# changzy00/pytorch-attention

Measured on AMD Instinct MI355X. Metric: forward images/sec through one step (+ ms/block), B=256 per GPU, 224x224-derived shapes, higher is better.
Workload: dtype f32/f16; 1 GPU; north-star step: C2 SE+CBAM+ECA, C3 ViT-Attn, C4 CSWin s1-4 + XCABlock + XCA, DA x2, Mixer, C5 ViT-Base fwd; B=256/GPU; precision=fp16-mfma, ranks_seen=1, gather=none (single rank), batch_per_gpu=256, parallelism=batch-shard x1, dist_backend=none, rccl_self_test=not run (single rank), distinct_gpus=1, full=off: --full adds calibration, roofline, per-block and CPU-baseline figures

## Files before the change

pytorch-attention_amd/csrc/attn.hip:

```cpp
#include "common.h"
#include "mma.h"
#include "bufops.h"
#include <type_traits>

namespace {

struct AttnArgs {
    const void* qkv;
    void* out;
    const float* lepe_w;
    const float* lepe_b;
    int L, Ctot, c0, heads;
    int koff, voff, oc0;
    int reso, Hsp, Wsp, nWx, nwin;
    int T;
    unsigned wsp_magic;
    float scale;
    int pre_scale;
};

struct AttnPair {
    AttnArgs a0, a1;
    int split;
};
struct AttnPairRg : AttnPair {
    unsigned* ovf;
};
struct AttnPairQ : AttnPair {
    int q_tiles, q_rows;
    int out_rows;
};
template <bool IO16, bool QLIM = false>
using attn_kargs = typename std::conditional<QLIM, AttnPairQ, typename std::conditional<IO16, AttnPair, AttnPairRg>::type>::type;
template <bool IO16>
const attn_kargs<IO16>& attn_pick(const AttnPairRg& p) { return p; }

#ifndef MI355_ATTN_FMA_SM
#define MI355_ATTN_FMA_SM 1
#endif
template <int PREC, int D, int KT, bool LEPE, bool IO16, int NW, int OCC = 1, int TFULL = -1, bool QLIM = false>
__global__ __launch_bounds__(NW * 64, OCC) void win_attn_kernel(const attn_kargs<IO16, QLIM> pr) {
    static_assert(!QLIM || (IO16 && !LEPE), "the query limit exists for the plain 16-bit-I/O core");
    constexpr bool FMA_SM = MI355_ATTN_FMA_SM != 0;
    const int lid = xcd_contiguous_block();
    const bool second = lid >= pr.split;
    const AttnArgs a = second ? pr.a1 : pr.a0;
    constexpr int NTHR = NW * 64;
    static_assert(!IO16 || PREC != 0, "16-bit I/O exists for the fp16 / bf16 operand modes only");
    using M_ = Mma<PREC>;
    using v8 = typename M_::v8;
    using v4 = typename M_::v4;
    using el = typename M_::e;
    constexpr int NS = M_::NSPLIT;
    constexpr int TK = KT * 16;
    constexpr int KP = D + 8;
    constexpr int VP = TK + 4;
    constexpr bool RG = !IO16 && PREC == 1;
    float rgm = 0.f;
    constexpr int OP = IO16 ? D + 8 : D + 4;
    constexpr int K_EL = TK * KP, V_EL = D * VP;
    using slab_t = typename std::conditional<IO16, unsigned short, float>::type;
    __shared__ __attribute__((aligned(16))) unsigned short s_k[NS * K_EL];
    __shared__ __attribute__((aligned(16))) unsigned short s_v[NS * V_EL];
    __shared__ __attribute__((aligned(16))) slab_t s_o[NW * 16 * OP];

    const int t = threadIdx.x, lane = t & 63, wave = t >> 6;
    int bid = lid - (second ? pr.split : 0);
    const int head = bid % a.heads; bid /= a.heads;
    const int win = bid % a.nwin;
    const int b = bid / a.nwin;
    const int T = a.T;
    const int wy0 = (win / a.nWx) * a.Hsp, wx0 = (win % a.nWx) * a.Wsp;
    const int ch0 = a.c0 + head * D;
    const int och0 = a.oc0 + head * D;
    const long row3 = 3L * a.Ctot;
    using gel = typename std::conditional<IO16, el, float>::type;
    const gel* base = static_cast<const gel*>(a.qkv) + (long)b * a.L * row3 + ch0;
    auto srow = [&](int s) { return a.Wsp == 1 ? s : (int)__umulhi((unsigned)s, a.wsp_magic); };
    auto tok = [&](int s) { const int r = srow(s); return (wy0 + r) * a.reso + wx0 + (s - r * a.Wsp); };

    const int l15 = lane & 15, g = lane >> 4;
    int nqt = (T + 15) >> 4;
    int qmax = T;
    if constexpr (QLIM) {
        nqt = pr.q_tiles < nqt ? pr.q_tiles : nqt;
        qmax = pr.q_rows < T ? pr.q_rows : T;
    }
    int orows = a.L;
    if constexpr (QLIM) orows = pr.out_rows;
    constexpr int NQ = (KT + NW - 1) / NW;
    const rsrc_t img_rs = make_rsrc(IO16 ? static_cast<const void*>(base) : nullptr, IO16 ? (bufops_u32)((long)a.L * row3 * sizeof(gel)) : 0u);
    auto ld16 = [&](bool live, int token, int el_off) -> v8 {
        const bufops_u32 off = live ? (bufops_u32)((token * (int)row3 + el_off) * 2) : OOB;
        return __builtin_bit_cast(v8, __builtin_amdgcn_raw_buffer_load_b128(img_rs, off, 0, 0));
    };
    v8 qraw[IO16 ? NQ : 1][D / 32];
    if constexpr (IO16) {
#pragma unroll
        for (int iq = 0; iq < NQ; ++iq) {
            const int qs = (wave + iq * NW) * 16 + l15;
            const int tq = tok(qs < T ? qs : 0);
            const bool ql = QLIM ? (qs < qmax && wave + iq * NW < nqt) : qs < T;
#pragma unroll
            for (int ks = 0; ks < D / 32; ++ks) qraw[iq][ks] = ld16(ql, tq, ks * 32 + g * 8);
        }
    }
    __shared__ float s_lw[LEPE ? D * 10 : 1];
    if constexpr (LEPE) {
        for (int q = t; q < D * 10; q += NTHR) {
            const int c = q / 10, i = q - c * 10;
            s_lw[q] = i < 9 ? a.lepe_w[(long)(head * D + c) * 9 + i] : a.lepe_b[head * D + c];
        }
    }

    constexpr int D4 = D / 4;
    if constexpr (IO16) {
        constexpr int D8 = D / 8;
        constexpr int NKI = (TK * D8 + NTHR - 1) / NTHR, NVI = ((TK / 4) * D8 + NTHR - 1) / NTHR;
        v8 kreg[NKI];
        v8 vreg[NVI][4];
#pragma unroll
        for (int it = 0; it < NKI; ++it) {
            const int idx = t + it * NTHR, key = idx / D8, d8 = idx % D8;
            const bool live = idx < TK * D8 && key < T;
            kreg[it] = ld16(live, tok(live ? key : 0), a.koff + d8 * 8);
        }
#pragma unroll
        for (int it = 0; it < NVI; ++it) {
            const int idx = t + it * NTHR, kg = idx / D8, d8 = idx % D8;
#pragma unroll
            for (int j = 0; j < 4; ++j) {
                const int key = kg * 4 + j;
                const bool live = idx < (TK / 4) * D8 && key < T;
                vreg[it][j] = ld16(live, tok(live ? key : 0), a.voff + d8 * 8);
            }
        }
#pragma unroll
        for (int it = 0; it < NKI; ++it) {
            const int idx = t + it * NTHR, key = idx / D8, d8 = idx % D8;
            if (idx < TK * D8) *reinterpret_cast<v8*>(s_k + key * KP + d8 * 8) = kreg[it];
        }
#pragma unroll
        for (int it = 0; it < NVI; ++it) {
            const int idx = t + it * NTHR, kg = idx / D8, d8 = idx % D8;
            if (idx < (TK / 4) * D8) {
#pragma unroll
                for (int q = 0; q < 8; ++q)
                    *reinterpret_cast<v4*>(s_v + (d8 * 8 + q) * VP + kg * 4) =
                        v4{vreg[it][0][q], vreg[it][1][q], vreg[it][2][q], vreg[it][3][q]};
            }
        }
    } else {
    for (int idx = t; idx < TK * D4; idx += NTHR) {
        const int key = idx / D4, d4 = idx % D4;
        f4 v = {0.f, 0.f, 0.f, 0.f};
        if (key < T) v = *reinterpret_cast<const f4*>(base + (long)tok(key) * row3 + a.koff + d4 * 4);
        if constexpr (RG) rgm = rg_absmax4(rgm, v);
        const v4 h = M_::cvt(v);
        *reinterpret_cast<v4*>(s_k + key * KP + d4 * 4) = h;
        if constexpr (NS == 2) *reinterpret_cast<v4*>(s_k + K_EL + key * KP + d4 * 4) = M_::cvt_lo(v, h);
    }
    for (int idx = t; idx < (TK / 4) * D4; idx += NTHR) {
        const int kg = idx / D4, d4 = idx % D4;
        f4 r[4];
#pragma unroll
        for (int j = 0; j < 4; ++j) {
            const int key = kg * 4 + j;
            r[j] = f4{0.f, 0.f, 0.f, 0.f};
            if (key < T) r[j] = *reinterpret_cast<const f4*>(base + (long)tok(key) * row3 + a.voff + d4 * 4);
            if constexpr (RG) rgm = rg_absmax4(rgm, r[j]);
        }
        const f4 c[4] = {{r[0].x, r[1].x, r[2].x, r[3].x}, {r[0].y, r[1].y, r[2].y, r[3].y},
                         {r[0].z, r[1].z, r[2].z, r[3].z}, {r[0].w, r[1].w, r[2].w, r[3].w}};
#pragma unroll
        for (int q = 0; q < 4; ++q) {
            const v4 h = M_::cvt(c[q]);
            *reinterpret_cast<v4*>(s_v + (d4 * 4 + q) * VP + kg * 4) = h;
            if constexpr (NS == 2) *reinterpret_cast<v4*>(s_v + V_EL + (d4 * 4 + q) * VP + kg * 4) = M_::cvt_lo(c[q], h);
        }
    }
    }
    __shared__ unsigned short s_tap[LEPE ? TK * 9 : 1];
    if constexpr (LEPE) {
        for (int q = t; q < NS * D; q += NTHR) s_v[(q / D) * V_EL + (q % D) * VP + TK] = 0;
        for (int q = t; q < T * 9; q += NTHR) {
            const int slot = q / 9, tap = q - slot * 9;
            const int ty = srow(slot), tx = slot - ty * a.Wsp;
            const int yy = ty + tap / 3 - 1, xx = tx + tap % 3 - 1;
            s_tap[q] = (unsigned short)(((yy >= 0 && yy < a.Hsp && xx >= 0 && xx < a.Wsp) ? yy * a.Wsp + xx : TK) * 2);
        }
    }
    __syncthreads();

    slab_t* slab = s_o + wave * 16 * OP;
#pragma unroll
    for (int iq = 0; iq < NQ; ++iq) {
        const int qt = wave + iq * NW;
        if (qt >= nqt) break;
        const int qs = qt * 16 + l15;
        v8 qf[D / 32][NS];
        {
            const gel* qrow = base + (long)tok(qs < T ? qs : 0) * row3;
#pragma unroll
            for (int ks = 0; ks < D / 32; ++ks) {
                f4 lo4 = {0.f, 0.f, 0.f, 0.f}, hi4 = {0.f, 0.f, 0.f, 0.f};
                if constexpr (IO16) {
                    const v8 raw = qraw[iq][ks];
                    if (!a.pre_scale) { qf[ks][0] = raw; continue; }
                    lo4 = f4{(float)raw[0], (float)raw[1], (float)raw[2], (float)raw[3]};
                    hi4 = f4{(float)raw[4], (float)raw[5], (float)raw[6], (float)raw[7]};
                } else if (qs < T) {
                    lo4 = *reinterpret_cast<const f4*>(qrow + ks * 32 + g * 8);
                    hi4 = *reinterpret_cast<const f4*>(qrow + ks * 32 + g * 8 + 4);
                }
                if (a.pre_scale) { lo4 = lo4 * a.scale; hi4 = hi4 * a.scale; }
                if constexpr (RG) rgm = rg_absmax4(rg_absmax4(rgm, lo4), hi4);
                const v4 h0 = M_::cvt(lo4), h1 = M_::cvt(hi4);
                qf[ks][0] = v8{h0.x, h0.y, h0.z, h0.w, h1.x, h1.y, h1.z, h1.w};
                if constexpr (NS == 2) {
                    const v4 e0 = M_::cvt_lo(lo4, h0), e1 = M_::cvt_lo(hi4, h1);
                    qf[ks][1] = v8{e0.x, e0.y, e0.z, e0.w, e1.x, e1.y, e1.z, e1.w};
                }
            }
        }
        f4 o[D / 16];
        float sum;
        const f4 zero4 = {0.f, 0.f, 0.f, 0.f};
        f4 s[KT];
#pragma unroll
        for (int kt = 0; kt < KT; ++kt) {
            f4 acc = zero4;
            if (kt < TFULL || kt * 16 < T) {
#pragma unroll
                for (int ks = 0; ks < D / 32; ++ks) {
                    v8 kf[NS];
#pragma unroll
                    for (int sp = 0; sp < NS; ++sp)
                        kf[sp] = *reinterpret_cast<const v8*>(s_k + sp * K_EL + (kt * 16 + l15) * KP + ks * 32 + g * 8);
                    acc = mma_step<PREC>(kf, qf[ks], acc);
                }
            }
            s[kt] = acc;
        }
        const float post = (a.pre_scale ? 1.0f : a.scale) * 1.44269504088896340736f;
        float m = -INFINITY;
        sum = 0.f;
        if constexpr (PREC != 0 && FMA_SM) {
#pragma unroll
            for (int kt = 0; kt < KT; ++kt)
#pragma unroll
                for (int r = 0; r < 4; ++r) {
                    const int key = kt * 16 + g * 4 + r;
                    const float v = (kt < TFULL || key < T) ? s[kt][r] : -INFINITY;
                    s[kt][r] = v;
                    m = fmaxf(m, v);
                }
            m = fmaxf(m, __shfl_xor(m, 16, WAVE));
            m = fmaxf(m, __shfl_xor(m, 32, WAVE));
            const float mneg = -(m * post);
#pragma unroll
            for (int kt = 0; kt < KT; ++kt)
#pragma unroll
                for (int r = 0; r < 4; ++r) {
                    s[kt][r] = __builtin_amdgcn_exp2f(__builtin_fmaf(s[kt][r], post, mneg));
                }
        } else {
#pragma unroll
            for (int kt = 0; kt < KT; ++kt)
#pragma unroll
                for (int r = 0; r < 4; ++r) {
                    const int key = kt * 16 + g * 4 + r;
                    const float v = (kt < TFULL || key < T) ? s[kt][r] * post : -INFINITY;
                    s[kt][r] = v;
                    m = fmaxf(m, v);
                }
            m = fmaxf(m, __shfl_xor(m, 16, WAVE));
            m = fmaxf(m, __shfl_xor(m, 32, WAVE));
#pragma unroll
            for (int kt = 0; kt < KT; ++kt)
#pragma unroll
                for (int r = 0; r < 4; ++r) {
                    const float p = __builtin_amdgcn_exp2f(s[kt][r] - m);
                    s[kt][r] = p;
                    sum += p;
                }
        }
        if constexpr (!(PREC != 0 && FMA_SM)) {
            sum += __shfl_xor(sum, 16, WAVE);
            sum += __shfl_xor(sum, 32, WAVE);
        }
#pragma unroll
        for (int nt = 0; nt < D / 16; ++nt) o[nt] = zero4;
        f4 osum = zero4;
        typedef typename M_::e el1_t;
        const v8 ones = v8{(el1_t)1.0f, (el1_t)1.0f, (el1_t)1.0f, (el1_t)1.0f, (el1_t)1.0f, (el1_t)1.0f, (el1_t)1.0f, (el1_t)1.0f};
#pragma unroll
        for (int kb = 0; kb < KT / 2; ++kb) {
            if (2 * kb < TFULL || kb * 32 < T) {
                v8 pf[NS];
                {
                    const f4 p0 = s[2 * kb], p1 = s[2 * kb + 1];
                    const v4 h0 = M_::cvt(p0), h1 = M_::cvt(p1);
                    pf[0] = v8{h0.x, h0.y, h0.z, h0.w, h1.x, h1.y, h1.z, h1.w};
                    if constexpr (NS == 2) {
                        const v4 e0 = M_::cvt_lo(p0, h0), e1 = M_::cvt_lo(p1, h1);
                        pf[1] = v8{e0.x, e0.y, e0.z, e0.w, e1.x, e1.y, e1.z, e1.w};
                    }
                }
#pragma unroll
                for (int nt = 0; nt < D / 16; ++nt) {
                    v8 vf[NS];
#pragma unroll
                    for (int sp = 0; sp < NS; ++sp) {
                        const unsigned short* vr = s_v + sp * V_EL + (nt * 16 + l15) * VP + kb * 32 + g * 4;
                        const v4 a0 = *reinterpret_cast<const v4*>(vr);
                        const v4 a1 = *reinterpret_cast<const v4*>(vr + 16);
                        vf[sp] = v8{a0.x, a0.y, a0.z, a0.w, a1.x, a1.y, a1.z, a1.w};
                    }
                    o[nt] = mma_step<PREC>(vf, pf, o[nt]);
                }
                if constexpr (PREC != 0 && FMA_SM) osum = M_::mma(ones, pf[0], osum);
            }
        }
        if constexpr (PREC != 0 && FMA_SM) sum = osum.x;
        const float inv = __builtin_amdgcn_rcpf(sum);
        int off[LEPE ? 9 : 1];
        bool qlive = false;
        if constexpr (LEPE) {
            const int qslot = qt * 16 + l15;
            qlive = qslot < T;
            const unsigned short* tp = s_tap + (qlive ? qslot : 0) * 9;
#pragma unroll
            for (int i = 0; i < 9; ++i) off[i] = tp[i];
        }
#pragma unroll
        for (int nt = 0; nt < D / 16; ++nt) {
            f4 val = o[nt] * inv;
            if constexpr (LEPE) {
                if (qlive) {
#pragma unroll
                    for (int r = 0; r < 4; ++r) {
                        const int d = nt * 16 + g * 4 + r;
                        const float* lwp = s_lw + d * 10;
                        const char* vrow = reinterpret_cast<const char*>(s_v + d * VP);
                        float acc = lwp[9];
#pragma unroll
                        for (int i = 0; i < 9; ++i) {
                            float vv = (float)(*reinterpret_cast<const el*>(vrow + off[i]));
                            if constexpr (NS == 2) vv += (float)(*reinterpret_cast<const el*>(vrow + V_EL * 2 + off[i]));
                            acc = __builtin_fmaf(lwp[i], vv, acc);
                        }
                        val[r] += acc;
                    }
                }
            }
            if constexpr (IO16) *reinterpret_cast<v4*>(slab + l15 * OP + nt * 16 + g * 4) = M_::cvt(val);
            else *reinterpret_cast<f4*>(slab + l15 * OP + nt * 16 + g * 4) = val;
        }
        __builtin_amdgcn_wave_barrier();
        __builtin_amdgcn_fence(__ATOMIC_ACQ_REL, "wavefront");
        if constexpr (IO16) {
            constexpr int LPR = D / 8, RPI = 64 / LPR;
#pragma unroll
            for (int it = 0; it < 16 / RPI; ++it) {
                const int r = it * RPI + lane / LPR, c8 = (lane % LPR) * 8;
                const int qslot = qt * 16 + r;
                if (QLIM ? qslot < qmax : qslot < T)
                    *reinterpret_cast<v8*>(static_cast<gel*>(a.out) + ((long)b * orows + tok(qslot)) * a.Ctot + och0 + c8) =
                        *reinterpret_cast<const v8*>(slab + r * OP + c8);
            }
        } else {
            constexpr int LPR = D / 4, RPI = 64 / LPR;
#pragma unroll
            for (int it = 0; it < 16 / RPI; ++it) {
                const int r = it * RPI + lane / LPR, c4 = (lane % LPR) * 4;
                const int qslot = qt * 16 + r;
                if (qslot < T)
                    *reinterpret_cast<f4*>(static_cast<gel*>(a.out) + ((long)b * a.L + tok(qslot)) * a.Ctot + och0 + c4) =
                        *reinterpret_cast<const f4*>(slab + r * OP + c4);
            }
        }
        __builtin_amdgcn_wave_barrier();
        __builtin_amdgcn_fence(__ATOMIC_ACQ_REL, "wavefront");
    }
    if constexpr (RG) rg_report(rgm, pr.ovf, 7u);
}

constexpr int LONG_KB = 8;
constexpr int LONG_TMAX = 512;
template <int PREC, int KT, bool IO16, int NW>
__global__ __launch_bounds__(NW * 64, 1) void win_attn_long_kernel(const attn_kargs<IO16> pr) {
    constexpr int D = 32, KB = LONG_KB;
    static_assert(!IO16 || PREC != 0, "16-bit I/O exists for the fp16 / bf16 operand modes only");
    static_assert(KT % 2 == 0 && KB % 2 == 0 && KT * 16 <= LONG_TMAX, "P.V consumes key tiles in pairs");
    const int lid = xcd_contiguous_block();
    const bool second = lid >= pr.split;
    const AttnArgs a = second ? pr.a1 : pr.a0;
    constexpr int NTHR = NW * 64;
    using M_ = Mma<PREC>;
    using v8 = typename M_::v8;
    using v4 = typename M_::v4;
    using el = typename M_::e;
    constexpr int NS = M_::NSPLIT;
    constexpr int TK = KT * 16;
    constexpr int KP = D + 8;
    constexpr int VP = TK + 4;
    static_assert((TK + 1) * 2 <= VP * 2 && VP * 2 < 65536, "tap byte offsets stay inside a V^T row");
    constexpr bool RG = !IO16 && PREC == 1;
    float rgm = 0.f;
    constexpr int OP = IO16 ? D + 8 : D + 4;
    constexpr int K_EL = TK * KP, V_EL = D * VP;
    using slab_t = typename std::conditional<IO16, unsigned short, float>::type;
    __shared__ __attribute__((aligned(16))) unsigned short s_k[NS * K_EL];
    __shared__ __attribute__((aligned(16))) unsigned short s_v[NS * V_EL];
    __shared__ __attribute__((aligned(16))) slab_t s_o[NW * 16 * OP];
    __shared__ float s_lw[D * 10];
    static_assert(sizeof(unsigned short) * NS * (K_EL + V_EL) + sizeof(slab_t) * NW * 16 * OP + sizeof(float) * D * 10 <= 163840,
                  "K, V^T, the output slab and the LePE weights share one workgroup's LDS");

    const int t = threadIdx.x, lane = t & 63, wave = t >> 6;
    int bid = lid - (second ? pr.split : 0);
    const int head = bid % a.heads; bid /= a.heads;
    const int win = bid % a.nwin;
    const int b = bid / a.nwin;
    const int T = a.T;
    const int wy0 = (win / a.nWx) * a.Hsp, wx0 = (win % a.nWx) * a.Wsp;
    const int ch0 = a.c0 + head * D;
    const int och0 = a.oc0 + head * D;
    const long row3 = 3L * a.Ctot;
    using gel = typename std::conditional<IO16, el, float>::type;
    const gel* base = static_cast<const gel*>(a.qkv) + (long)b * a.L * row3 + ch0;
    auto srow = [&](int s) { return a.Wsp == 1 ? s : (int)__umulhi((unsigned)s, a.wsp_magic); };
    auto tok = [&](int s) { const int r = srow(s); return (wy0 + r) * a.reso + wx0 + (s - r * a.Wsp); };

    const int l15 = lane & 15, g = lane >> 4;
    const int nqt = (T + 15) >> 4;
    const rsrc_t img_rs = make_rsrc(IO16 ? static_cast<const void*>(base) : nullptr, IO16 ? (bufops_u32)((long)a.L * row3 * sizeof(gel)) : 0u);
    auto ld16 = [&](bool live, int token, int el_off) -> v8 {
        const bufops_u32 off = live ? (bufops_u32)((token * (int)row3 + el_off) * 2) : OOB;
        return __builtin_bit_cast(v8, __builtin_amdgcn_raw_buffer_load_b128(img_rs, off, 0, 0));
    };
    const f4 zero4 = {0.f, 0.f, 0.f, 0.f};
    struct QF32 { f4 lo, hi; };
    using qraw_t = typename std::conditional<IO16, v8, QF32>::type;
    auto ldq = [&](int qt_) -> qraw_t {
        const int qs = qt_ * 16 + l15;
        const bool live = qs < T;
        const int tq = tok(live ? qs : 0);
        if constexpr (IO16) {
            return ld16(live, tq, g * 8);
        } else {
            QF32 r{zero4, zero4};
            if (live) {
                const float* qrow = base + (long)tq * row3 + g * 8;
                r.lo = *reinterpret_cast<const f4*>(qrow);
                r.hi = *reinterpret_cast<const f4*>(qrow + 4);
            }
            return r;
        }
    };
    qraw_t qnext = ldq(wave);
    for (int q = t; q < D * 10; q += NTHR) {
        const int c = q / 10, i = q - c * 10;
        s_lw[q] = i < 9 ? a.lepe_w[(long)(head * D + c) * 9 + i] : a.lepe_b[head * D + c];
    }

    constexpr int D4 = D / 4;
    if constexpr (IO16) {
        constexpr int D8 = D / 8;
        constexpr int NKI = (TK * D8 + NTHR - 1) / NTHR, NVI = ((TK / 4) * D8 + NTHR - 1) / NTHR;
        v8 kreg[NKI];
        v8 vreg[NVI][4];
#pragma unroll
        for (int it = 0; it < NKI; ++it) {
            const int idx = t + it * NTHR, key = idx / D8, d8 = idx % D8;
            const bool live = idx < TK * D8 && key < T;
            kreg[it] = ld16(live, tok(live ? key : 0), a.koff + d8 * 8);
        }
#pragma unroll
        for (int it = 0; it < NVI; ++it) {
            const int idx = t + it * NTHR, kg = idx / D8, d8 = idx % D8;
#pragma unroll
            for (int j = 0; j < 4; ++j) {
                const int key = kg * 4 + j;
                const bool live = idx < (TK / 4) * D8 && key < T;
                vreg[it][j] = ld16(live, tok(live ? key : 0), a.voff + d8 * 8);
            }
        }
#pragma unroll
        for (int it = 0; it < NKI; ++it) {
            const int idx = t + it * NTHR, key = idx / D8, d8 = idx % D8;
            if (idx < TK * D8) *reinterpret_cast<v8*>(s_k + key * KP + d8 * 8) = kreg[it];
        }
#pragma unroll
        for (int it = 0; it < NVI; ++it) {
            const int idx = t + it * NTHR, kg = idx / D8, d8 = idx % D8;
            if (idx < (TK / 4) * D8) {
#pragma unroll
                for (int q = 0; q < 8; ++q)
                    *reinterpret_cast<v4*>(s_v + (d8 * 8 + q) * VP + kg * 4) =
                        v4{vreg[it][0][q], vreg[it][1][q], vreg[it][2][q], vreg[it][3][q]};
            }
        }
    } else {
        for (int idx = t; idx < TK * D4; idx += NTHR) {
            const int key = idx / D4, d4 = idx % D4;
            f4 v = zero4;
            if (key < T) v = *reinterpret_cast<const f4*>(base + (long)tok(key) * row3 + a.koff + d4 * 4);
            if constexpr (RG) rgm = rg_absmax4(rgm, v);
            const v4 h = M_::cvt(v);
            *reinterpret_cast<v4*>(s_k + key * KP + d4 * 4) = h;
            if constexpr (NS == 2) *reinterpret_cast<v4*>(s_k + K_EL + key * KP + d4 * 4) = M_::cvt_lo(v, h);
        }
        for (int idx = t; idx < (TK / 4) * D4; idx += NTHR) {
            const int kg = idx / D4, d4 = idx % D4;
            f4 r[4];
#pragma unroll
            for (int j = 0; j < 4; ++j) {
                const int key = kg * 4 + j;
                r[j] = zero4;
                if (key < T) r[j] = *reinterpret_cast<const f4*>(base + (long)tok(key) * row3 + a.voff + d4 * 4);
                if constexpr (RG) rgm = rg_absmax4(rgm, r[j]);
            }
            const f4 c[4] = {{r[0].x, r[1].x, r[2].x, r[3].x}, {r[0].y, r[1].y, r[2].y, r[3].y},
                             {r[0].z, r[1].z, r[2].z, r[3].z}, {r[0].w, r[1].w, r[2].w, r[3].w}};
#pragma unroll
            for (int q = 0; q < 4; ++q) {
                const v4 h = M_::cvt(c[q]);
                *reinterpret_cast<v4*>(s_v + (d4 * 4 + q) * VP + kg * 4) = h;
                if constexpr (NS == 2) *reinterpret_cast<v4*>(s_v + V_EL + (d4 * 4 + q) * VP + kg * 4) = M_::cvt_lo(c[q], h);
            }
        }
    }
    for (int q = t; q < NS * D; q += NTHR) s_v[(q / D) * V_EL + (q % D) * VP + TK] = 0;
    __syncthreads();

    slab_t* slab = s_o + wave * 16 * OP;
    const float post = (a.pre_scale ? 1.0f : a.scale) * 1.44269504088896340736f;
    for (int qt = wave; qt < nqt; qt += NW) {
        const qraw_t qr = qnext;
        qnext = ldq(qt + NW);
        v8 qf[NS];
        {
            f4 lo4, hi4;
            if constexpr (IO16) {
                lo4 = f4{(float)qr[0], (float)qr[1], (float)qr[2], (float)qr[3]};
                hi4 = f4{(float)qr[4], (float)qr[5], (float)qr[6], (float)qr[7]};
            } else {
                lo4 = qr.lo; hi4 = qr.hi;
            }
            if (a.pre_scale) { lo4 = lo4 * a.scale; hi4 = hi4 * a.scale; }
            if constexpr (RG) rgm = rg_absmax4(rg_absmax4(rgm, lo4), hi4);
            const v4 h0 = M_::cvt(lo4), h1 = M_::cvt(hi4);
            qf[0] = v8{h0.x, h0.y, h0.z, h0.w, h1.x, h1.y, h1.z, h1.w};
            if constexpr (NS == 2) {
                const v4 e0 = M_::cvt_lo(lo4, h0), e1 = M_::cvt_lo(hi4, h1);
                qf[1] = v8{e0.x, e0.y, e0.z, e0.w, e1.x, e1.y, e1.z, e1.w};
            }
        }
        f4 o[D / 16] = {zero4, zero4};
        float m = -INFINITY, sum = 0.f;
        typedef typename M_::e el1_t;
        const v8 ones = v8{(el1_t)1.0f, (el1_t)1.0f, (el1_t)1.0f, (el1_t)1.0f, (el1_t)1.0f, (el1_t)1.0f, (el1_t)1.0f, (el1_t)1.0f};
        for (int kb0 = 0; kb0 * 16 < T; kb0 += KB) {
            f4 s[KB];
#pragma unroll
            for (int kt = 0; kt < KB; ++kt) {
                f4 acc = zero4;
                if ((kb0 + kt) * 16 < T) {
                    v8 kf[NS];
#pragma unroll
                    for (int sp = 0; sp < NS; ++sp)
                        kf[sp] = *reinterpret_cast<const v8*>(s_k + sp * K_EL + ((kb0 + kt) * 16 + l15) * KP + g * 8);
                    acc = mma_step<PREC>(kf, qf, acc);
                }
                s[kt] = acc;
            }
            float mb = -INFINITY;
#pragma unroll
            for (int kt = 0; kt < KB; ++kt)
#pragma unroll
                for (int r = 0; r < 4; ++r) {
                    const int key = (kb0 + kt) * 16 + g * 4 + r;
                    const float sc = PREC != 0 ? s[kt][r] : s[kt][r] * post;
                    const float v = key < T ? sc : -INFINITY;
                    s[kt][r] = v;
                    mb = fmaxf(mb, v);
                }
            mb = fmaxf(mb, __shfl_xor(mb, 16, WAVE));
            mb = fmaxf(mb, __shfl_xor(mb, 32, WAVE));
            const float mn = fmaxf(m, mb);
            float alpha, bsum = 0.f;
            if constexpr (PREC != 0) {
                const float mneg = -(mn * post);
                alpha = m == -INFINITY ? 0.f : __builtin_amdgcn_exp2f(__builtin_fmaf(m, post, mneg));
#pragma unroll
                for (int kt = 0; kt < KB; ++kt)
#pragma unroll
                    for (int r = 0; r < 4; ++r) s[kt][r] = __builtin_amdgcn_exp2f(__builtin_fmaf(s[kt][r], post, mneg));
            } else {
                alpha = m == -INFINITY ? 0.f : __builtin_amdgcn_exp2f(m - mn);
#pragma unroll
                for (int kt = 0; kt < KB; ++kt)
#pragma unroll
                    for (int r = 0; r < 4; ++r) {
                        const float p = __builtin_amdgcn_exp2f(s[kt][r] - mn);
                        s[kt][r] = p;
                        bsum += p;
                    }
            }
            m = mn;
#pragma unroll
            for (int nt = 0; nt < D / 16; ++nt) o[nt] = o[nt] * alpha;
            f4 osum = zero4;
#pragma unroll
            for (int kb = 0; kb < KB / 2; ++kb) {
                if ((kb0 + 2 * kb) * 16 < T) {
                    v8 pf[NS];
                    {
                        const f4 p0 = s[2 * kb], p1 = s[2 * kb + 1];
                        const v4 h0 = M_::cvt(p0), h1 = M_::cvt(p1);
                        pf[0] = v8{h0.x, h0.y, h0.z, h0.w, h1.x, h1.y, h1.z, h1.w};
                        if constexpr (NS == 2) {
                            const v4 e0 = M_::cvt_lo(p0, h0), e1 = M_::cvt_lo(p1, h1);
                            pf[1] = v8{e0.x, e0.y, e0.z, e0.w, e1.x, e1.y, e1.z, e1.w};
                        }
                    }
#pragma unroll
                    for (int nt = 0; nt < D / 16; ++nt) {
                        v8 vf[NS];
#pragma unroll
                        for (int sp = 0; sp < NS; ++sp) {
                            const unsigned short* vr = s_v + sp * V_EL + (nt * 16 + l15) * VP + (kb0 + 2 * kb) * 16 + g * 4;
                            const v4 a0 = *reinterpret_cast<const v4*>(vr);
                            const v4 a1 = *reinterpret_cast<const v4*>(vr + 16);
                            vf[sp] = v8{a0.x, a0.y, a0.z, a0.w, a1.x, a1.y, a1.z, a1.w};
                        }
                        o[nt] = mma_step<PREC>(vf, pf, o[nt]);
                    }
                    if constexpr (PREC != 0) osum = M_::mma(ones, pf[0], osum);
                }
            }
            if constexpr (PREC != 0) bsum = osum.x;
            sum = sum * alpha + bsum;
        }
        if constexpr (PREC == 0) {
            sum += __shfl_xor(sum, 16, WAVE);
            sum += __shfl_xor(sum, 32, WAVE);
        }
        const float inv = __builtin_amdgcn_rcpf(sum);
        const int qslot = qt * 16 + l15;
        const bool qlive = qslot < T;
        int off[9];
        {
            const int ty = srow(qlive ? qslot : 0), tx = (qlive ? qslot : 0) - ty * a.Wsp;
#pragma unroll
            for (int i = 0; i < 9; ++i) {
                const int yy = ty + i / 3 - 1, xx = tx + i % 3 - 1;
                off[i] = ((yy >= 0 && yy < a.Hsp && xx >= 0 && xx < a.Wsp) ? yy * a.Wsp + xx : TK) * 2;
            }
        }
#pragma unroll
        for (int nt = 0; nt < D / 16; ++nt) {
            f4 val = o[nt] * inv;
            if (qlive) {
#pragma unroll
                for (int r = 0; r < 4; ++r) {
                    const int d = nt * 16 + g * 4 + r;
                    const float* lwp = s_lw + d * 10;
                    const char* vrow = reinterpret_cast<const char*>(s_v + d * VP);
                    float acc = lwp[9];
#pragma unroll
                    for (int i = 0; i < 9; ++i) {
                        float vv = (float)(*reinterpret_cast<const el*>(vrow + off[i]));
                        if constexpr (NS == 2) vv += (float)(*reinterpret_cast<const el*>(vrow + V_EL * 2 + off[i]));
                        acc = __builtin_fmaf(lwp[i], vv, acc);
                    }
                    val[r] += acc;
                }
            }
            if constexpr (IO16) *reinterpret_cast<v4*>(slab + l15 * OP + nt * 16 + g * 4) = M_::cvt(val);
            else *reinterpret_cast<f4*>(slab + l15 * OP + nt * 16 + g * 4) = val;
        }
        __builtin_amdgcn_wave_barrier();
        __builtin_amdgcn_fence(__ATOMIC_ACQ_REL, "wavefront");
        if constexpr (IO16) {
            constexpr int LPR = D / 8, RPI = 64 / LPR;
#pragma unroll
            for (int it = 0; it < 16 / RPI; ++it) {
                const int r = it * RPI + lane / LPR, c8 = (lane % LPR) * 8;
                const int qs = qt * 16 + r;
                if (qs < T)
                    *reinterpret_cast<v8*>(static_cast<gel*>(a.out) + ((long)b * a.L + tok(qs)) * a.Ctot + och0 + c8) =
                        *reinterpret_cast<const v8*>(slab + r * OP + c8);
            }
        } else {
            constexpr int LPR = D / 4, RPI = 64 / LPR;
#pragma unroll
            for (int it = 0; it < 16 / RPI; ++it) {
                const int r = it * RPI + lane / LPR, c4 = (lane % LPR) * 4;
                const int qs = qt * 16 + r;
                if (qs < T)
                    *reinterpret_cast<f4*>(static_cast<gel*>(a.out) + ((long)b * a.L + tok(qs)) * a.Ctot + och0 + c4) =
                        *reinterpret_cast<const f4*>(slab + r * OP + c4);
            }
        }
        __builtin_amdgcn_wave_barrier();
        __builtin_amdgcn_fence(__ATOMIC_ACQ_REL, "wavefront");
    }
    if constexpr (RG) rg_report(rgm, pr.ovf, 7u);
}

template <bool IO16>
int launch_attn_long(const AttnPairRg& pr, int grid, int B, int precision, hipStream_t st) {
    const AttnArgs& a = pr.a0;
    const int Tmax = pr.split < grid && pr.a1.T > a.T ? pr.a1.T : a.T;
    if (Tmax > LONG_TMAX) return mi355::fail(MI355_EUNSUPPORTED, "LePE attention: %d tokens per stripe window > %d", Tmax, LONG_TMAX);
    if (IO16 && (long)a.L * 3L * a.Ctot * 2L >= (1L << 31))
        return mi355::fail(MI355_EUNSUPPORTED, "LePE attention, 16-bit I/O: the qkv rows of one image span %ld bytes (limit 2^31)", (long)a.L * 3L * a.Ctot * 2L);
    MI355_TRACE(st, "win_attn_long_kernel<d=32,lepe%s> B=%d windows=%d heads=%d tokens=%d", IO16 ? ",io16" : "", B, a.nwin, a.heads, a.T);
#define GOL(P, KT_, NW_) win_attn_long_kernel<P, KT_, (IO16 && P != 0), NW_><<<grid, NW_ * 64, 0, st>>>(attn_pick<(IO16 && P != 0)>(pr))
#define BYT(P) do { if (Tmax <= 320) GOL(P, 20, 8); else GOL(P, 32, (P == 0 ? 4 : 8)); } while (0)
    switch (precision) {
        case MI355_PREC_STRICT: BYT(0); break;
        case MI355_PREC_FP16:   BYT(1); break;
        case MI355_PREC_BF16:   BYT(2); break;
        default: return mi355::fail(MI355_EINVAL, "precision must be 0, 1 or 2 (got %d)", precision);
    }
#undef BYT
#undef GOL
    return MI355_OK;
}

template <int D, bool LEPE, bool IO16>
int launch_attn(const AttnArgs& a, int B, int precision, hipStream_t st, const AttnArgs* other = nullptr) {
    AttnPairRg pr{};
    pr.a0 = a;
    pr.split = B * a.nwin * a.heads;
    int grid = pr.split;
    if (other) {
        pr.a1 = *other;
        grid += B * other->nwin * other->heads;
    }
    if (IO16 && precision == MI355_PREC_STRICT)
        return mi355::fail(MI355_EINVAL, "16-bit activation I/O needs precision 1 (fp16) or 2 (bf16)");
    if (!IO16 && precision == MI355_PREC_FP16) pr.ovf = mi355::range_word(st);
    if constexpr (LEPE && D == 32) {
        if (a.T > 224 || (other && other->T > 224)) return launch_attn_long<IO16>(pr, grid, B, precision, st);
    }
    MI355_TRACE(st, "win_attn_kernel<d=%d%s%s> B=%d windows=%d heads=%d tokens=%d", D, LEPE ? ",lepe" : "", IO16 ? ",io16" : "", B, a.nwin, a.heads, a.T);
#define GO(P, KT_, NW_) win_attn_kernel<P, D, KT_, LEPE, (IO16 && P != 0), NW_><<<grid, NW_ * 64, 0, st>>>(attn_pick<(IO16 && P != 0)>(pr))
#define GO_OCC(P, KT_, NW_, OCC_) win_attn_kernel<P, D, KT_, LEPE, (IO16 && P != 0), NW_, ((IO16 && P != 0 && D == 32) ? OCC_ : 1)><<<grid, NW_ * 64, 0, st>>>(attn_pick<(IO16 && P != 0)>(pr))
#define GO_FULL(P, KT_, NW_, OCC_, TF_) \
    win_attn_kernel<P, D, KT_, LEPE, (IO16 && P != 0), NW_, ((IO16 && P != 0 && D == 32) ? OCC_ : 1), TF_><<<grid, NW_ * 64, 0, st>>>(attn_pick<(IO16 && P != 0)>(pr))
    const bool hot = IO16 && (!other || other->T == a.T);
#define BYKT(P)                                          \
    do {                                                 \
        if (a.T <= 64) { if (hot && P != 0 && a.T >= 48) GO_FULL(P, 4, 4, 6, 3); else GO_OCC(P, 4, 4, 6); }          \
        else if (a.T <= 128) { if (hot && P != 0 && a.T >= 96) GO_FULL(P, 8, 4, 5, 6); else GO_OCC(P, 8, 4, 5); }    \
        else if (IO16 && P != 0) {                                                                                    \
             \
                                \
            if (a.T >= 192 && a.T <= 208 && mi355::opt(mi355::O_ATTN_NW) == 7) GO_FULL(P, 14, 7, 1, 12);                          \
            else if (a.T >= 192) GO_FULL(P, 14, 8, 1, 12); else GO(P, 14, 8); }                                          \
        else GO(P, 14, 4);                               \
    } while (0)
    switch (precision) {
        case MI355_PREC_STRICT: BYKT(0); break;
        case MI355_PREC_FP16:   BYKT(1); break;
        case MI355_PREC_BF16:   BYKT(2); break;
        default: return mi355::fail(MI355_EINVAL, "precision must be 0, 1 or 2 (got %d)", precision);
    }
#undef BYKT
#undef GO_FULL
#undef GO_OCC
#undef GO
    return MI355_OK;
}

template <int D>
int launch_attn_rows(const AttnArgs& a, int B, int q_rows, int out_rows, int precision, hipStream_t st) {
    AttnPairQ pr{};
    pr.a0 = a;
    pr.split = B * a.nwin * a.heads;
    pr.q_rows = q_rows;
    pr.q_tiles = (q_rows + 15) >> 4;
    pr.out_rows = out_rows;
    const int grid = pr.split;
    MI355_TRACE(st, "win_attn_kernel<d=%d,io16,rows> B=%d heads=%d tokens=%d q_rows=%d", D, B, a.heads, a.T, q_rows);
#define GOQ(P, KT_, NW_) win_attn_kernel<P, D, KT_, false, true, NW_, 1, -1, true><<<grid, NW_ * 64, 0, st>>>(pr)
#define BYKTQ(P) do { if (a.T <= 64) GOQ(P, 4, 4); else if (a.T <= 128) GOQ(P, 8, 4); else GOQ(P, 14, 8); } while (0)
    if (precision == MI355_PREC_FP16) BYKTQ(1); else BYKTQ(2);
#undef BYKTQ
#undef GOQ
    return MI355_OK;
}

}

static AttnArgs sdpa_args(const void* qkv, void* out, int N, int heads, int d, float scale) {
    AttnArgs a{};
    a.qkv = qkv; a.out = out; a.L = N; a.Ctot = heads * d; a.c0 = 0; a.heads = heads;
    a.koff = a.Ctot; a.voff = 2 * a.Ctot; a.oc0 = 0;
    a.reso = N; a.Hsp = 1; a.Wsp = N; a.nWx = 1; a.nwin = 1; a.T = N; a.scale = scale; a.pre_scale = 0;
    a.wsp_magic = (unsigned)(((1ull << 32) + (unsigned)N - 1) / (unsigned)N);
    return a;
}

static int sdpa_common(const void* qkv, void* out, int B, int N, int heads, int d, float scale, int precision, bool io16,
                       hipStream_t st) {
    const AttnArgs a = sdpa_args(qkv, out, N, heads, d, scale);
    if (d == 64) return io16 ? launch_attn<64, false, true>(a, B, precision, st) : launch_attn<64, false, false>(a, B, precision, st);
    return io16 ? launch_attn<32, false, true>(a, B, precision, st) : launch_attn<32, false, false>(a, B, precision, st);
}

static AttnArgs lepe_args(const void* qkv, const float* getv_w, const float* getv_b, void* out, int reso, int Ctot, int c0, int heads,
                          int Hsp, int Wsp, float scale) {
    AttnArgs a{};
    a.qkv = qkv; a.out = out; a.lepe_w = getv_w; a.lepe_b = getv_b;
    a.L = reso * reso; a.Ctot = Ctot; a.c0 = c0; a.heads = heads;
    a.koff = Ctot; a.voff = 2 * Ctot; a.oc0 = c0;
    a.reso = reso; a.Hsp = Hsp; a.Wsp = Wsp; a.nWx = reso / Wsp; a.nwin = (reso / Hsp) * (reso / Wsp); a.T = Hsp * Wsp;
    a.scale = scale; a.pre_scale = 1;
    a.wsp_magic = (unsigned)(((1ull << 32) + (unsigned)Wsp - 1) / (unsigned)Wsp);
    return a;
}

static int lepe_common(const void* qkv, const float* getv_w, const float* getv_b, void* out, int B, int reso, int Ctot, int c0, int Cb,
                       int heads, int Hsp, int Wsp, float scale, int precision, bool io16, hipStream_t st) {
    (void)Cb;
    const AttnArgs a = lepe_args(qkv, getv_w, getv_b, out, reso, Ctot, c0, heads, Hsp, Wsp, scale);
    return io16 ? launch_attn<32, true, true>(a, B, precision, st) : launch_attn<32, true, false>(a, B, precision, st);
}

#define SDPA_CHECKS(fn)                                                                                                   \
    MI355_CHECK_ARG(qkv && out && B > 0 && N > 0 && heads > 0);                                                           \
    if (!(d == 32 || d == 64)) return mi355::fail(MI355_EUNSUPPORTED, fn ": head dim %d (built: 32, 64)", d);            \
    if (N > 224) return mi355::fail(MI355_EUNSUPPORTED, fn ": sequence length %d > 224 (single-pass softmax core)", N);   \
    MI355_CHECK_ARG(aligned16(qkv) && aligned16(out))

#define LEPE_CHECKS(fn)                                                                                                    \
    MI355_CHECK_ARG(qkv && getv_w && getv_b && out);                                                                       \
    MI355_CHECK_ARG(B > 0 && reso > 0 && Ctot > 0 && c0 >= 0 && Cb > 0 && c0 + Cb <= Ctot && heads > 0 && Cb % heads == 0); \
    MI355_CHECK_ARG(Hsp > 0 && Wsp > 0 && reso % Hsp == 0 && reso % Wsp == 0);                                             \
    if (Cb / heads != 32) return mi355::fail(MI355_EUNSUPPORTED, fn ": head dim %d (built: 32)", Cb / heads);             \
    if (Hsp * Wsp > 512) return mi355::fail(MI355_EUNSUPPORTED, fn ": %d tokens per stripe window > 512", Hsp * Wsp);     \
    MI355_CHECK_ARG((Ctot & 7) == 0 && (c0 & 7) == 0 && aligned16(qkv) && aligned16(out))

extern "C" {

int mi355_sdpa_fwd(const float* qkv, float* out, int B, int N, int heads, int d, float scale, int precision,
                   mi355_stream_t stream) {
    SDPA_CHECKS("mi355_sdpa_fwd");
    int rc = sdpa_common(qkv, out, B, N, heads, d, scale, precision, false, static_cast<hipStream_t>(stream));
    if (rc) return rc;
    MI355_LAUNCH_CHECK();
    return MI355_OK;
}

int mi355_sdpa16_fwd(const void* qkv, void* out, int B, int N, int heads, int d, float scale, int precision,
                     mi355_stream_t stream) {
    SDPA_CHECKS("mi355_sdpa16_fwd");
    int rc = sdpa_common(qkv, out, B, N, heads, d, scale, precision, true, static_cast<hipStream_t>(stream));
    if (rc) return rc;
    MI355_LAUNCH_CHECK();
    return MI355_OK;
}

int mi355_sdpa16_rows_fwd(const void* qkv, void* out, int B, int N, int heads, int d, float scale, int q_rows, int out_rows, int precision,
                          mi355_stream_t stream) {
    SDPA_CHECKS("mi355_sdpa16_rows_fwd");
    MI355_CHECK_ARG(q_rows > 0 && q_rows <= N && out_rows >= q_rows);
    MI355_CHECK_ARG(precision == MI355_PREC_FP16 || precision == MI355_PREC_BF16);
    const AttnArgs a = sdpa_args(qkv, out, N, heads, d, scale);
    hipStream_t st = static_cast<hipStream_t>(stream);
    if (d == 64) launch_attn_rows<64>(a, B, q_rows, out_rows, precision, st);
    else         launch_attn_rows<32>(a, B, q_rows, out_rows, precision, st);
    MI355_LAUNCH_CHECK();
    return MI355_OK;
}

int mi355_cswin_lepe_attn_fwd(const float* qkv, const float* getv_w, const float* getv_b, float* out, int B, int reso, int Ctot,
                              int c0, int Cb, int heads, int Hsp, int Wsp, float scale, int precision, mi355_stream_t stream) {
    LEPE_CHECKS("mi355_cswin_lepe_attn_fwd");
    int rc = lepe_common(qkv, getv_w, getv_b, out, B, reso, Ctot, c0, Cb, heads, Hsp, Wsp, scale, precision, false,
                         static_cast<hipStream_t>(stream));
    if (rc) return rc;
    MI355_LAUNCH_CHECK();
    return MI355_OK;
}

int mi355_cswin_lepe_attn16_pair_fwd(const void* qkv, const float* getv_w0, const float* getv_b0, const float* getv_w1, const float* getv_b1,
                                     void* out, int B, int reso, int Ctot, int heads, int split, float scale, int precision,
                                     mi355_stream_t stream) {
    MI355_CHECK_ARG(qkv && getv_w0 && getv_b0 && getv_w1 && getv_b1 && out);
    MI355_CHECK_ARG(B > 0 && reso > 0 && Ctot > 0 && heads > 0 && (Ctot / 2) % heads == 0 && split > 0 && reso % split == 0);
    if (Ctot / 2 / heads != 32) return mi355::fail(MI355_EUNSUPPORTED, "mi355_cswin_lepe_attn16_pair_fwd: head dim %d (built: 32)", Ctot / 2 / heads);
    if (reso * split > 512) return mi355::fail(MI355_EUNSUPPORTED, "mi355_cswin_lepe_attn16_pair_fwd: %d tokens per stripe window > 512", reso * split);
    MI355_CHECK_ARG((Ctot & 15) == 0 && aligned16(qkv) && aligned16(out));
    const AttnArgs a0 = lepe_args(qkv, getv_w0, getv_b0, out, reso, Ctot, 0, heads, reso, split, scale);
    const AttnArgs a1 = lepe_args(qkv, getv_w1, getv_b1, out, reso, Ctot, Ctot / 2, heads, split, reso, scale);
    int rc = launch_attn<32, true, true>(a0, B, precision, static_cast<hipStream_t>(stream), &a1);
    if (rc) return rc;
    MI355_LAUNCH_CHECK();
    return MI355_OK;
}

int mi355_cswin_lepe_attn16_fwd(const void* qkv, const float* getv_w, const float* getv_b, void* out, int B, int reso, int Ctot,
                                int c0, int Cb, int heads, int Hsp, int Wsp, float scale, int precision, mi355_stream_t stream) {
    LEPE_CHECKS("mi355_cswin_lepe_attn16_fwd");
    int rc = lepe_common(qkv, getv_w, getv_b, out, B, reso, Ctot, c0, Cb, heads, Hsp, Wsp, scale, precision, true,
                         static_cast<hipStream_t>(stream));
    if (rc) return rc;
    MI355_LAUNCH_CHECK();
    return MI355_OK;
}

}
```

Before: 16350 images/s.

## Swizzle K and permute V^T in LDS for conflict-free single b128 fragment reads

Replaces the padded linear LDS layouts for K and transposed V in the windowed attention core with an XOR-swizzled K image and a key-permuted, row-swizzled V^T image for non-LePE variants. The V fragment can then be fetched with one 128-bit LDS read instead of two 64-bit reads, and both fragment reads are meant to avoid bank conflicts. Compile-time checks verify the mapping is a bijection and that LDS usage still allows the intended occupancy. LePE variants keep the linear layout, and the added index arithmetic could cost some ALU work or make the staging writes conflict.

```diff
diff --git a/pytorch-attention_amd/csrc/attn.hip b/pytorch-attention_amd/csrc/attn.hip
--- a/pytorch-attention_amd/csrc/attn.hip
+++ b/pytorch-attention_amd/csrc/attn.hip
@@ -1,9 +1,12 @@
 #include "common.h"
 #include "mma.h"
 #include "bufops.h"
+#include "attn_lds.h"
 #include <type_traits>
 
 namespace {
+
+namespace L = attn_lds;
 
 struct AttnArgs {
     const void* qkv;
@@ -53,16 +56,21 @@
     using el = typename M_::e;
     constexpr int NS = M_::NSPLIT;
     constexpr int TK = KT * 16;
-    constexpr int KP = D + 8;
-    constexpr int VP = TK + 4;
+    using IM = typename std::conditional<LEPE, L::Linear<D>, L::Packed<D>>::type;
+    constexpr int VP = IM::vt_pitch(TK);
     constexpr bool RG = !IO16 && PREC == 1;
     float rgm = 0.f;
     constexpr int OP = IO16 ? D + 8 : D + 4;
-    constexpr int K_EL = TK * KP, V_EL = D * VP;
+    constexpr int K_EL = IM::k_elems(TK), V_EL = IM::vt_elems(TK);
     using slab_t = typename std::conditional<IO16, unsigned short, float>::type;
     __shared__ __attribute__((aligned(16))) unsigned short s_k[NS * K_EL];
     __shared__ __attribute__((aligned(16))) unsigned short s_v[NS * V_EL];
     __shared__ __attribute__((aligned(16))) slab_t s_o[NW * 16 * OP];
+    static_assert(L::image_ok_v<IM, TK>, "Packed: both fragment reads are conflict-free ds_read_b128 and the V^T key map is a bijection (attn_lds.h)");
+    static_assert(L::core_bytes<IM>(TK, NS, NW, IO16, LEPE, true) * OCC <= L::CU_BYTES, "OCC workgroups of this core share a CU's LDS");
+    static_assert(!(D == 64 && KT == 14 && NW == 8 && IO16 && !LEPE) ||
+                      (L::core_bytes<IM>(TK, NS, NW, IO16, LEPE, true) == 77824 && 2 * 77824 <= L::CU_BYTES),
+                  "the ViT core keeps two workgroups per CU");
 
     const int t = threadIdx.x, lane = t & 63, wave = t >> 6;
     int bid = lid - (second ? pr.split : 0);
@@ -80,6 +88,9 @@
     auto tok = [&](int s) { const int r = srow(s); return (wy0 + r) * a.reso + wx0 + (s - r * a.Wsp); };
 
     const int l15 = lane & 15, g = lane >> 4;
+    int kfo[D / 32];
+#pragma unroll
+    for (int ks = 0; ks < D / 32; ++ks) kfo[ks] = IM::k_chunk(l15, ks * 4 + g);
     int nqt = (T + 15) >> 4;
     int qmax = T;
     if constexpr (QLIM) {
@@ -138,7 +149,7 @@
 #pragma unroll
         for (int it = 0; it < NKI; ++it) {
             const int idx = t + it * NTHR, key = idx / D8, d8 = idx % D8;
-            if (idx < TK * D8) *reinterpret_cast<v8*>(s_k + key * KP + d8 * 8) = kreg[it];
+            if (idx < TK * D8) *reinterpret_cast<v8*>(s_k + IM::k_chunk(key, d8)) = kreg[it];
         }
 #pragma unroll
         for (int it = 0; it < NVI; ++it) {
@@ -146,7 +157,7 @@
             if (idx < (TK / 4) * D8) {
 #pragma unroll
                 for (int q = 0; q < 8; ++q)
-                    *reinterpret_cast<v4*>(s_v + (d8 * 8 + q) * VP + kg * 4) =
+                    *reinterpret_cast<v4*>(s_v + IM::vt_row(d8 * 8 + q) * VP + IM::vt_pos(kg * 4)) =
                         v4{vreg[it][0][q], vreg[it][1][q], vreg[it][2][q], vreg[it][3][q]};
             }
         }
@@ -157,8 +168,8 @@
         if (key < T) v = *reinterpret_cast<const f4*>(base + (long)tok(key) * row3 + a.koff + d4 * 4);
         if constexpr (RG) rgm = rg_absmax4(rgm, v);
         const v4 h = M_::cvt(v);
-        *reinterpret_cast<v4*>(s_k + key * KP + d4 * 4) = h;
-        if constexpr (NS == 2) *reinterpret_cast<v4*>(s_k + K_EL + key * KP + d4 * 4) = M_::cvt_lo(v, h);
+        *reinterpret_cast<v4*>(s_k + IM::k_at(key, d4 * 4)) = h;
+        if constexpr (NS == 2) *reinterpret_cast<v4*>(s_k + K_EL + IM::k_at(key, d4 * 4)) = M_::cvt_lo(v, h);
     }
     for (int idx = t; idx < (TK / 4) * D4; idx += NTHR) {
         const int kg = idx / D4, d4 = idx % D4;
@@ -175,19 +186,19 @@
 #pragma unroll
         for (int q = 0; q < 4; ++q) {
             const v4 h = M_::cvt(c[q]);
-            *reinterpret_cast<v4*>(s_v + (d4 * 4 + q) * VP + kg * 4) = h;
-            if constexpr (NS == 2) *reinterpret_cast<v4*>(s_v + V_EL + (d4 * 4 + q) * VP + kg * 4) = M_::cvt_lo(c[q], h);
+            *reinterpret_cast<v4*>(s_v + IM::vt_row(d4 * 4 + q) * VP + IM::vt_pos(kg * 4)) = h;
+            if constexpr (NS == 2) *reinterpret_cast<v4*>(s_v + V_EL + IM::vt_row(d4 * 4 + q) * VP + IM::vt_pos(kg * 4)) = M_::cvt_lo(c[q], h);
         }
     }
     }
     __shared__ unsigned short s_tap[LEPE ? TK * 9 : 1];
     if constexpr (LEPE) {
-        for (int q = t; q < NS * D; q += NTHR) s_v[(q / D) * V_EL + (q % D) * VP + TK] = 0;
+        for (int q = t; q < NS * D; q += NTHR) s_v[(q / D) * V_EL + (q % D) * VP + IM::vt_zero(TK)] = 0;
         for (int q = t; q < T * 9; q += NTHR) {
             const int slot = q / 9, tap = q - slot * 9;
             const int ty = srow(slot), tx = slot - ty * a.Wsp;
             const int yy = ty + tap / 3 - 1, xx = tx + tap % 3 - 1;
-            s_tap[q] = (unsigned short)(((yy >= 0 && yy < a.Hsp && xx >= 0 && xx < a.Wsp) ? yy * a.Wsp + xx : TK) * 2);
+            s_tap[q] = (unsigned short)(((yy >= 0 && yy < a.Hsp && xx >= 0 && xx < a.Wsp) ? IM::vt_pos(yy * a.Wsp + xx) : IM::vt_zero(TK)) * 2);
         }
     }
     __syncthreads();
@@ -236,7 +247,7 @@
                     v8 kf[NS];
 #pragma unroll
                     for (int sp = 0; sp < NS; ++sp)
-                        kf[sp] = *reinterpret_cast<const v8*>(s_k + sp * K_EL + (kt * 16 + l15) * KP + ks * 32 + g * 8);
+                        kf[sp] = *reinterpret_cast<const v8*>(s_k + sp * K_EL + IM::k_tile(kt) + kfo[ks]);
                     acc = mma_step<PREC>(kf, qf[ks], acc);
                 }
             }
@@ -312,10 +323,14 @@
                     v8 vf[NS];
 #pragma unroll
                     for (int sp = 0; sp < NS; ++sp) {
-                        const unsigned short* vr = s_v + sp * V_EL + (nt * 16 + l15) * VP + kb * 32 + g * 4;
-                        const v4 a0 = *reinterpret_cast<const v4*>(vr);
-                        const v4 a1 = *reinterpret_cast<const v4*>(vr + 16);
-                        vf[sp] = v8{a0.x, a0.y, a0.z, a0.w, a1.x, a1.y, a1.z, a1.w};
+                        const unsigned short* vr = s_v + sp * V_EL + IM::vt_row(nt * 16 + l15) * VP + IM::vt_frag(kb, g);
+                        if constexpr (IM::one_read) {
+                            vf[sp] = *reinterpret_cast<const v8*>(vr);
+                        } else {
+                            const v4 a0 = *reinterpret_cast<const v4*>(vr);
+                            const v4 a1 = *reinterpret_cast<const v4*>(vr + 16);
+                            vf[sp] = v8{a0.x, a0.y, a0.z, a0.w, a1.x, a1.y, a1.z, a1.w};
+                        }
                     }
                     o[nt] = mma_step<PREC>(vf, pf, o[nt]);
                 }
@@ -342,7 +357,7 @@
                     for (int r = 0; r < 4; ++r) {
                         const int d = nt * 16 + g * 4 + r;
                         const float* lwp = s_lw + d * 10;
-                        const char* vrow = reinterpret_cast<const char*>(s_v + d * VP);
+                        const char* vrow = reinterpret_cast<const char*>(s_v + IM::vt_row(d) * VP);
                         float acc = lwp[9];
 #pragma unroll
                         for (int i = 0; i < 9; ++i) {
diff --git a/pytorch-attention_amd/csrc/attn_lds.h b/pytorch-attention_amd/csrc/attn_lds.h
--- /dev/null
+++ b/pytorch-attention_amd/csrc/attn_lds.h
@@ -0,0 +1,170 @@
+#pragma once
+
+namespace attn_lds {
+
+template <int D>
+constexpr int k_swz(int key) {
+    static_assert(D == 32 || D == 64, "swizzles exist for head widths 32 and 64");
+    return D == 64 ? (key & 7) : 3 * ((key >> 3) & 1);
+}
+template <int D>
+constexpr int k_chunk(int key, int chunk) { return key * D + ((chunk ^ k_swz<D>(key)) << 3); }
+template <int D>
+constexpr int k_at(int key, int d) { return k_chunk<D>(key, d >> 3) + (d & 7); }
+template <int D>
+constexpr int k_tile(int kt) { return kt * 16 * D; }
+template <int D>
+constexpr int k_elems(int TK) { return TK * D; }
+
+constexpr int vt_pitch(int TK) { return TK + 16; }
+constexpr int vt_pos(int key) { return (key & ~31) + (((key >> 2) & 3) << 3) + (((key >> 4) & 1) << 2) + (key & 3); }
+constexpr int vt_frag(int kb, int g) { return kb * 32 + g * 8; }
+constexpr int vt_zero(int TK) { return TK; }
+constexpr int vt_row(int d) { return d ^ (((d >> 4) & 1) << 1) ^ ((d >> 5) & 1); }
+constexpr int vt_elems(int D, int TK) { return D * vt_pitch(TK); }
+
+constexpr int frag_key(int kb, int g, int j) { return kb * 32 + (j >> 2) * 16 + g * 4 + (j & 3); }
+
+constexpr bool vt_map_ok(int TK) {
+    if (TK % 32 != 0 || TK > 512 || vt_pitch(TK) % 8 != 0 || vt_zero(TK) >= vt_pitch(TK)) return false;
+    bool seen[512] = {};
+    for (int key = 0; key < TK; ++key) {
+        const int p = vt_pos(key);
+        if (p < 0 || p >= TK || seen[p]) return false;
+        seen[p] = true;
+    }
+    for (int kb = 0; kb < TK / 32; ++kb)
+        for (int g = 0; g < 4; ++g)
+            for (int j = 0; j < 8; ++j)
+                if (vt_pos(frag_key(kb, g, j)) != vt_frag(kb, g) + j) return false;
+    return true;
+}
+
+constexpr int b128_group(int lane) {
+    const int w = lane & 31;
+    const bool first = w < 4 || (w >= 12 && w < 16) || (w >= 20 && w < 28);
+    return (lane >> 5) * 2 + (first ? 0 : 1);
+}
+constexpr int b128_cycles(const int (&addr)[64]) {
+    int seen[4][16][16] = {};
+    int n[4][16] = {};
+    for (int lane = 0; lane < 64; ++lane) {
+        if (addr[lane] < 0 || addr[lane] % 16 != 0) return -1;
+        const int grp = b128_group(lane), slot = (addr[lane] / 16) % 16;
+        bool dup = false;
+        for (int i = 0; i < n[grp][slot]; ++i) dup = dup || seen[grp][slot][i] == addr[lane];
+        if (!dup) seen[grp][slot][n[grp][slot]++] = addr[lane];
+    }
+    int total = 0;
+    for (int grp = 0; grp < 4; ++grp) {
+        int worst = 0;
+        for (int slot = 0; slot < 16; ++slot) worst = n[grp][slot] > worst ? n[grp][slot] : worst;
+        total += worst;
+    }
+    return total;
+}
+template <int D>
+constexpr int k_frag_cycles(int TK) {
+    int worst = 0;
+    for (int kt = 0; kt < TK / 16; ++kt)
+        for (int ks = 0; ks < D / 32; ++ks) {
+            int addr[64] = {};
+            for (int lane = 0; lane < 64; ++lane) addr[lane] = 2 * k_chunk<D>(kt * 16 + (lane & 15), ks * 4 + (lane >> 4));
+            const int c = b128_cycles(addr);
+            if (c < 0) return -1;
+            worst = c > worst ? c : worst;
+        }
+    return worst;
+}
+constexpr int vt_frag_cycles(int D, int TK) {
+    int worst = 0;
+    for (int nt = 0; nt < D / 16; ++nt)
+        for (int kb = 0; kb < TK / 32; ++kb) {
+            int addr[64] = {};
+            for (int lane = 0; lane < 64; ++lane) addr[lane] = 2 * (vt_row(nt * 16 + (lane & 15)) * vt_pitch(TK) + vt_frag(kb, lane >> 4));
+            const int c = b128_cycles(addr);
+            if (c < 0) return -1;
+            worst = c > worst ? c : worst;
+        }
+    return worst;
+}
+constexpr int b64_write_cycles(const int (&addr)[64]) {
+    int total = 0;
+    for (int grp = 0; grp < 4; ++grp) {
+        int seen[16][16] = {}, n[16] = {}, worst = 0;
+        for (int lane = grp * 16; lane < grp * 16 + 16; ++lane) {
+            if (addr[lane] < 0 || addr[lane] % 8 != 0) return -1;
+            const int slot = (addr[lane] / 8) % 16;
+            bool dup = false;
+            for (int i = 0; i < n[slot]; ++i) dup = dup || seen[slot][i] == addr[lane];
+            if (!dup) seen[slot][n[slot]++] = addr[lane];
+            worst = n[slot] > worst ? n[slot] : worst;
+        }
+        total += worst;
+    }
+    return total;
+}
+template <typename RowFn>
+constexpr int vt_stage_cycles(int D, int TK, int pitch, RowFn row) {
+    int worst = 0;
+    for (int w = 0; w * 64 < (TK / 4) * (D / 8); ++w)
+        for (int q = 0; q < 8; ++q) {
+            int addr[64] = {};
+            for (int lane = 0; lane < 64; ++lane) {
+                const int idx = w * 64 + lane, kg = idx / (D / 8) % (TK / 4), d8 = idx % (D / 8);
+                addr[lane] = 2 * (row(d8 * 8 + q) * pitch + vt_pos(kg * 4));
+            }
+            const int c = b64_write_cycles(addr);
+            if (c < 0) return -1;
+            worst = c > worst ? c : worst;
+        }
+    return worst;
+}
+struct VtRow { constexpr int operator()(int d) const { return vt_row(d); } };
+struct PlainRow { constexpr int operator()(int d) const { return d; } };
+template <int D>
+constexpr bool image_ok(int TK) { return vt_map_ok(TK) && k_frag_cycles<D>(TK) == 4 && vt_frag_cycles(D, TK) == 4; }
+
+template <int D_>
+struct Packed {
+    static constexpr int D = D_;
+    static constexpr bool one_read = true;
+    static constexpr int k_chunk(int key, int chunk) { return attn_lds::k_chunk<D>(key, chunk); }
+    static constexpr int k_at(int key, int d) { return attn_lds::k_at<D>(key, d); }
+    static constexpr int k_tile(int kt) { return attn_lds::k_tile<D>(kt); }
+    static constexpr int k_elems(int TK) { return attn_lds::k_elems<D>(TK); }
+    static constexpr int vt_pitch(int TK) { return attn_lds::vt_pitch(TK); }
+    static constexpr int vt_pos(int key) { return attn_lds::vt_pos(key); }
+    static constexpr int vt_row(int d) { return attn_lds::vt_row(d); }
+    static constexpr int vt_frag(int kb, int g) { return attn_lds::vt_frag(kb, g); }
+    static constexpr int vt_zero(int TK) { return attn_lds::vt_zero(TK); }
+    static constexpr int vt_elems(int TK) { return attn_lds::vt_elems(D, TK); }
+    static constexpr bool ok(int TK) { return image_ok<D>(TK); }
+};
+template <int D_>
+struct Linear {
+    static constexpr int D = D_;
+    static constexpr bool one_read = false;
+    static constexpr int k_chunk(int key, int chunk) { return key * (D + 8) + chunk * 8; }
+    static constexpr int k_at(int key, int d) { return key * (D + 8) + d; }
+    static constexpr int k_tile(int kt) { return kt * 16 * (D + 8); }
+    static constexpr int k_elems(int TK) { return TK * (D + 8); }
+    static constexpr int vt_pitch(int TK) { return TK + 4; }
+    static constexpr int vt_pos(int key) { return key; }
+    static constexpr int vt_row(int d) { return d; }
+    static constexpr int vt_frag(int kb, int g) { return kb * 32 + g * 4; }
+    static constexpr int vt_zero(int TK) { return TK; }
+    static constexpr int vt_elems(int TK) { return D * (TK + 4); }
+    static constexpr bool ok(int TK) { return TK % 32 == 0 && TK <= 512; }
+};
+template <class IM, int TK>
+constexpr bool image_ok_v = IM::ok(TK);
+
+template <class IM>
+constexpr int core_bytes(int TK, int planes, int waves, bool io16, bool lepe, bool tap_table) {
+    return 2 * planes * (IM::k_elems(TK) + IM::vt_elems(TK)) + waves * 16 * (io16 ? (IM::D + 8) * 2 : (IM::D + 4) * 4) +
+           (lepe ? IM::D * 10 * 4 : 0) + (lepe && tap_table ? TK * 9 * 2 : 0);
+}
+constexpr int CU_BYTES = 163840;
+
+}
```

Result: no change. 16410 images/s, median of 5 (+0.4%).
